# IndigoPurple/DEQSCI

Hardware: AMD Instinct MI355X
Metric: reconstructed frames/sec at 256x256x8, 180 DEQ iters (higher is better)
Workload: dtype f32 (tensors and accumulation; the 64->64 layers' products as split-fp16 MFMAs, see arithmetic)

## Files before the change

deqsci_amd/_hip.py:

```python
import ctypes
import math
import os

import torch

LAYOUT_HWB = 0
LAYOUT_BHW = 1
MAX_M = 8
PART_STRIDE = MAX_M + 1
WGRAD_CHAIN = 4096

_LIB_PATH = os.environ.get("DEQSCI_HIP_LIB") or os.path.join(os.path.dirname(os.path.abspath(__file__)), "lib", "libdeqsci_hip.so")
_lib = None

_i64, _int, _f32, _ptr = ctypes.c_int64, ctypes.c_int, ctypes.c_float, ctypes.c_void_p
_f64 = ctypes.c_double

SIGNATURES = {
    "deqsci_sci_forward_f32": [_ptr, _ptr, _ptr, _i64, _i64, _i64, _i64, _int, _int, _ptr],
    "deqsci_sci_adjoint_f32": [_ptr, _ptr, _ptr, _i64, _i64, _i64, _i64, _int, _int, _ptr],
    "deqsci_phi_sum_f32": [_ptr, _ptr, _i64, _i64, _i64, _i64, _int, _ptr],
    "deqsci_gap_update_f32": [_ptr, _ptr, _ptr, _ptr, _ptr, _i64, _i64, _i64, _i64, _int, _int, _int, _ptr],
    "deqsci_gap_update_grad_f32": [_ptr, _ptr, _ptr, _ptr, _ptr, _ptr, _ptr, _ptr, _ptr, _i64, _i64, _i64, _i64, _int, _int, _ptr],
    "deqsci_sci_mask_grad_f32": [_ptr, _ptr, _ptr, _i64, _i64, _i64, _i64, _int, _int, _ptr],
# ... 34 lines not shown
    "deqsci_conv3x3_c64_to_1_split16": [_ptr, _ptr, _ptr, _i64, _i64, _i64, _int, _ptr, _int, _ptr],
    "deqsci_conv3x3_c64_to_1_p32": [_ptr, _ptr, _ptr, _i64, _i64, _i64, _int, _ptr, _int, _ptr],
    "deqsci_conv3x3_c1_to_64_p32": [_ptr, _ptr, _ptr, _i64, _i64, _i64, _int, _ptr, _int, _ptr, _ptr],
    "deqsci_ffdnet_head_p32": [_ptr, _ptr, _ptr, _i64, _ptr, _i64, _i64, _i64, _int, _ptr, _int, _ptr, _int, _ptr],
    "deqsci_ffdnet_tail_p32": [_ptr, _ptr, _ptr, _i64, _i64, _i64, _int, _ptr, _int, _ptr],
    "deqsci_conv3x3_c1_to_64_sp16": [_ptr, _ptr, _ptr, _i64, _i64, _i64, _int, _ptr, _int, _ptr, _ptr],
    "deqsci_ssim_f32": [_ptr, _ptr, _ptr, _i64, _i64, _i64, _i64, _int, _int, _int, _int, _ptr, _ptr],
    "deqsci_sqerr_rows_f32": [_ptr, _ptr, _ptr, _i64, _i64, _i64, _int, _ptr, _ptr],
    "deqsci_gaptv_f32": [_ptr, _ptr, _ptr, _ptr, _i64, _i64, _i64, _i64, _int, _int, _f64, _f64, _f64, _int, _ptr, _ptr, _ptr],
    "deqsci_tv_chambolle_f32": [_ptr, _ptr, _i64, _i64, _i64, _f64, _f64, _int, _f64, _ptr, _ptr, _ptr],
    "deqsci_relu_mask_pack_f32": [_ptr, _ptr, _i64, _ptr],
    "deqsci_conv3x3_c64_winograd_masked_f32": [_ptr, _ptr, _ptr, _ptr, _i64, _i64, _i64, _ptr],
    "deqsci_conv3x3_c1_to_64_masked_f32": [_ptr, _ptr, _ptr, _ptr, _i64, _i64, _i64, _ptr],
    "deqsci_ffdnet_head_masked_f32": [_ptr, _ptr, _ptr, _ptr, _i64, _i64, _i64, _ptr],
    "deqsci_power_step_f32": [_ptr, _ptr, _ptr, _ptr, _i64, _i64, _ptr, _ptr],
    "deqsci_broyden_dots_f32": [_ptr, _ptr, _ptr, _ptr, _ptr, _ptr, _ptr, _i64, _i64, _int, _int, _ptr],
    "deqsci_broyden_update_f32": [_ptr, _ptr, _ptr, _ptr, _ptr, _ptr, _ptr, _ptr, _ptr, _ptr, _i64, _i64, _int, _int, _int, _ptr],
    "deqsci_epsilon2_norms_f32": [_ptr, _ptr, _ptr, _ptr, _ptr, _i64, _i64, _ptr],
    "deqsci_epsilon2_update_f32": [_ptr, _ptr, _ptr, _ptr, _ptr, _ptr, _i64, _i64, _f32, _ptr],
    "deqsci_wgrad3x3_c64_c64_f32": [_ptr, _ptr, _ptr, _i64, _i64, _i64, _ptr, _ptr],
    "deqsci_wgrad3x3_c1_c64_f32": [_ptr, _ptr, _ptr, _int, _i64, _i64, _i64, _ptr, _ptr],
    "deqsci_wgrad3x3_c64_c64_bn_f32": [_ptr, _ptr, _ptr, _ptr, _ptr, _ptr, _ptr, _i64, _i64, _i64, _ptr, _ptr],
    "deqsci_wgrad3x3_shuffle_f32": [_ptr, _ptr, _i64, _ptr, _ptr, _int, _i64, _i64, _i64, _ptr, _ptr],
    "deqsci_realsn_power_f32": [_ptr, _ptr, _ptr, _ptr, _ptr, _int, _f32, _f32, _i64, _i64, _i64, _i64, _ptr, _ptr],
    "deqsci_realsn_grad_f32": [_ptr, _ptr, _ptr, _ptr, _ptr, _ptr, _f32, _i64, _i64, _i64, _i64, _ptr, _ptr],
    "deqsci_event_create": [ctypes.POINTER(_ptr)],
    "deqsci_event_destroy": [_ptr],
    "deqsci_event_elapsed_ms": [_ptr, _ptr, ctypes.POINTER(_f32)],
}
OTHER_EXPORTS = ("deqsci_version", "deqsci_error_string", "deqsci_anderson_chunks",
                 "deqsci_partials_bytes", "deqsci_gram_bytes", "deqsci_gram_ref_bytes", "deqsci_ssim_workspace_bytes",
                 "deqsci_gaptv_workspace_bytes", "deqsci_tv_chambolle_workspace_bytes", "deqsci_sqerr_workspace_bytes", "deqsci_power_workspace_bytes",
                 "deqsci_broyden_workspace_bytes", "deqsci_broyden_chunk", "deqsci_epsilon2_workspace_bytes", "deqsci_epsilon2_chunk",
                 "deqsci_wgrad_workspace_bytes", "deqsci_wgrad_bn_workspace_bytes", "deqsci_realsn_workspace_bytes")


class DeqsciHipError(RuntimeError):
    pass


def lib_path():
    return _LIB_PATH


def load():
    global _lib
    if _lib is not None:
        return _lib
    if not os.path.exists(_LIB_PATH):
        raise DeqsciHipError(
            f"{_LIB_PATH} is missing: build it with `make` (or __graft_entry__.build()). "
            "deqsci_amd has no CPU / eager fallback for its HIP kernels.")
    lib = ctypes.CDLL(_LIB_PATH, mode=ctypes.RTLD_GLOBAL)
    for name, argtypes in SIGNATURES.items():
        fn = getattr(lib, name)
        fn.argtypes = argtypes
        fn.restype = _int
    lib.deqsci_version.restype = ctypes.c_char_p
    lib.deqsci_error_string.restype = ctypes.c_char_p
    lib.deqsci_error_string.argtypes = [_int]
    lib.deqsci_anderson_chunks.restype = _i64
    lib.deqsci_anderson_chunks.argtypes = [_i64, _i64]
    lib.deqsci_partials_bytes.restype = ctypes.c_size_t
    lib.deqsci_partials_bytes.argtypes = [_i64, _i64]
    lib.deqsci_gram_bytes.restype = ctypes.c_size_t
    lib.deqsci_gram_bytes.argtypes = [_i64]
    lib.deqsci_gram_ref_bytes.restype = ctypes.c_size_t
    lib.deqsci_gram_ref_bytes.argtypes = [_i64, _i64]
    lib.deqsci_ssim_workspace_bytes.restype = _i64
    lib.deqsci_ssim_workspace_bytes.argtypes = [_i64, _i64, _i64, _i64, _int]
    lib.deqsci_sqerr_workspace_bytes.restype = ctypes.c_size_t
    lib.deqsci_sqerr_workspace_bytes.argtypes = [_i64, _i64]
    lib.deqsci_power_workspace_bytes.restype = ctypes.c_size_t
    lib.deqsci_power_workspace_bytes.argtypes = [_i64, _i64]
    lib.deqsci_broyden_workspace_bytes.restype = ctypes.c_size_t
    lib.deqsci_broyden_workspace_bytes.argtypes = [_i64, _i64, _int]
    lib.deqsci_broyden_chunk.restype = _i64
    lib.deqsci_broyden_chunk.argtypes = []
    lib.deqsci_epsilon2_workspace_bytes.restype = ctypes.c_size_t
    lib.deqsci_epsilon2_workspace_bytes.argtypes = [_i64, _i64]
    lib.deqsci_epsilon2_chunk.restype = _i64
    lib.deqsci_epsilon2_chunk.argtypes = []
    lib.deqsci_wgrad_workspace_bytes.restype = ctypes.c_size_t
    lib.deqsci_wgrad_workspace_bytes.argtypes = [_i64, _i64, _i64]
    lib.deqsci_wgrad_bn_workspace_bytes.restype = ctypes.c_size_t
    lib.deqsci_wgrad_bn_workspace_bytes.argtypes = [_i64, _i64, _i64]
    lib.deqsci_realsn_workspace_bytes.restype = ctypes.c_size_t
    lib.deqsci_realsn_workspace_bytes.argtypes = [_i64, _i64, _i64, _i64]
    lib.deqsci_gaptv_workspace_bytes.restype = _i64
# ... 793 lines not shown

def ffdnet_head_split16(x, weights, sigma, out=None, in_rng=None, in_exp=SP16_DEFAULT_EXP, out_rng=None, out_exp=SP16_DEFAULT_EXP, track=None):
    return _ffdnet_head("ffdnet_head_split16", Sp16, x, weights, sigma, out, in_rng, in_exp, out_rng, out_exp, track)


def _ffdnet_head(what, act, x, weights, sigma, out, in_rng, in_exp, out_rng, out_exp, track=None):
    n, c, H2, W2 = x.shape
    if c != 1 or H2 % 2 or W2 % 2 or not isinstance(weights, HeadSplit16Weights):
        raise DeqsciHipError(f"{what}: (n,1,even,even) image and HeadSplit16Weights required, got {tuple(x.shape)}")
    if sigma.numel() not in (1, n) or sigma.dtype != torch.float32 or not sigma.is_cuda:
        raise DeqsciHipError(f"{what}: sigma must be a fp32 GPU tensor with 1 or n elements")
    H, W = H2 // 2, W2 // 2
    o = out if out is not None else act.empty(n, H, W, x.device)
    if not isinstance(o, act) or (o.n, o.H, o.W) != (n, H, W):
        raise DeqsciHipError(f"{what}: out must be a {act.__name__} of the output's shape")
    o.rng, o.exp = out_rng, int(out_exp)
    wp = weights.packed if weights.packed.device == x.device else weights.packed.to(x.device)
    args = (_p(x, "x"), wp.data_ptr(), sigma.data_ptr(), 0 if sigma.numel() == 1 else sigma.stride(0), o.t.data_ptr(), n, H, W, weights.sw,
            _rng(in_rng, n), int(in_exp), _rng(out_rng, n), o.exp)
    with _dev(x):
        if act is Sp16:
            _check(load().deqsci_ffdnet_head_split16(*args, _rng(track, n), _stream()), what)
        else:
            _check(load().deqsci_ffdnet_head_p32(*args, _stream()), what)
    return o


def tail_split16(h, weights, out=None):
    if not isinstance(h, Sp16):
        raise DeqsciHipError("tail_split16: an Sp16 activation and TailSplit16Weights are required")
    return _tail("tail_split16", h, weights, out)


def _tail(what, h, weights, out):
    if not isinstance(weights, TailSplit16Weights):
        raise DeqsciHipError(f"{what}: TailSplit16Weights of a (4,64,3,3) or (1,64,3,3) weight are required")
    f = 2 if weights.cout == 4 else 1
    o = out if out is not None else torch.empty((h.n, 1, f * h.H, f * h.W), device=h.t.device, dtype=torch.float32)
    wp = weights.packed if weights.packed.device == h.t.device else weights.packed.to(h.t.device)
    if isinstance(h, Sp16):
        fn = load().deqsci_ffdnet_tail_split16 if weights.cout == 4 else load().deqsci_conv3x3_c64_to_1_split16
    else:
        fn = load().deqsci_ffdnet_tail_p32 if weights.cout == 4 else load().deqsci_conv3x3_c64_to_1_p32
    with _dev(h.t):
        _check(fn(h.t.data_ptr(), wp.data_ptr(), _p(o, "out"), h.n, h.H, h.W, weights.sw, _rng(h.rng, h.n), h.exp, _stream()), what)
    return o


def conv3x3_c64_split16(x, weights, bias=None, relu=True, out=None, out_f32=False, events=None, out_rng=None, out_exp=SP16_DEFAULT_EXP,
                        track=None):
    if not isinstance(x, Sp16) or tuple(x.t.shape) != (x.n, 4, 2, 2, x.H, x.W, 8) or not x.t.is_contiguous() or x.t.dtype != torch.float16 or not x.t.is_cuda:
        raise DeqsciHipError("conv3x3_c64_split16: a contiguous Sp16 GPU activation is required")
    if not isinstance(weights, Split16Weights) or weights.packed.numel() != 4 * 9 * 2 * 2 * 64 * 8:
        raise DeqsciHipError("conv3x3_c64_split16: weights must be a Split16Weights")
    n, H, W, dev = x.n, x.H, x.W, x.t.device
    wp = weights.packed if weights.packed.device == dev else weights.packed.to(dev)
    if track is not None:
        if out_f32:
            raise DeqsciHipError("conv3x3_c64_split16: a measuring launch (track=) serves the sp16 output")
        with _dev(x.t):
            _check(load().deqsci_conv3x3_c64_split16(x.t.data_ptr(), wp.data_ptr(), _p(bias, "bias", True), None, n, H, W, 1 if relu else 0,
                                                     weights.sw, _rng(x.rng, n), x.exp, None, 0, _rng(track, n), 0, _stream(), None, None),
                   "conv3x3_c64_split16 (measuring)")
        return None
    if out_f32:
        o = out if out is not None else torch.empty((n, 64, H, W), dtype=torch.float32, device=dev, memory_format=torch.channels_last)
        ot = o
    else:
        o = out if out is not None else Sp16.empty(n, H, W, dev)
        o.rng, o.exp = out_rng, int(out_exp)
        ot = o.t
    ev = _hook_events("s16", n, H, W, events) or (None, None)
    with _dev(x.t):
        _check(load().deqsci_conv3x3_c64_split16(x.t.data_ptr(), wp.data_ptr(), _p(bias, "bias", True), ot.data_ptr(), n, H, W, 1 if relu else 0,
                                                 weights.sw, _rng(x.rng, n), x.exp, _rng(out_rng, n), int(out_exp), None, 1 if out_f32 else 0,
                                                 _stream(), ev[0], ev[1]), "conv3x3_c64_split16")
# ... 169 lines not shown
        p = torch.stack((hi, lo), 0)
        p = p.reshape(2, 3, 2, 2, 2, 32, 4, 2, 8)
        self.packed = p.permute(6, 2, 3, 1, 0, 4, 7, 5, 8).contiguous()


def _act_check(x, what):
    if (not isinstance(x, P32) or tuple(x.t.shape) != (x.n, 8, 2, x.H, -(-x.W // 64), 2, 32, 4) or x.t.dtype != torch.float32 or not x.t.is_contiguous()
            or not x.t.is_cuda):
        raise DeqsciHipError(f"{what}: a contiguous P32 GPU activation is required")


def conv3x3_c64_wino16(x, weights, bias=None, relu=True, out=None, events=None, out_rng=None, out_exp=SP16_DEFAULT_EXP):
    _act_check(x, "conv3x3_c64_wino16")
    if not isinstance(weights, Wino16Weights) or weights.packed.numel() != 4 * 2 * 2 * 3 * 2 * 2 * 64 * 8:
        raise DeqsciHipError("conv3x3_c64_wino16: weights must be a Wino16Weights")
    n, H, W, dev = x.n, x.H, x.W, x.t.device
    wp = weights.packed if weights.packed.device == dev else weights.packed.to(dev)
    o = out if out is not None else P32.empty(n, H, W, dev)
    if not isinstance(o, P32):
        raise DeqsciHipError("conv3x3_c64_wino16: out must be a P32")
    o.rng, o.exp = out_rng, int(out_exp)
    ev = _hook_events("w16", n, H, W, events) or (None, None)
    with _dev(x.t):
        _check(load().deqsci_conv3x3_c64_wino16(x.t.data_ptr(), wp.data_ptr(), _p(bias, "bias", True), o.t.data_ptr(), n, H, W, 1 if relu else 0,
                                                weights.sw, _rng(x.rng, n), x.exp, _rng(out_rng, n), int(out_exp), _stream(), ev[0], ev[1]),
               "conv3x3_c64_wino16")
    return o


def ffdnet_head_p32(x, weights, sigma, out=None, in_rng=None, in_exp=SP16_DEFAULT_EXP, out_rng=None, out_exp=SP16_DEFAULT_EXP):
    return _ffdnet_head("ffdnet_head_p32", P32, x, weights, sigma, out, in_rng, in_exp, out_rng, out_exp)


def ffdnet_tail_p32(h, weights, out=None):
    _act_check(h, "ffdnet_tail_p32")
    return _tail("ffdnet_tail_p32", h, weights, out)


def conv3x3_c64_wino16_stack(x, stack, ranges=None, events=None, per_launch=None, rng_offset=0, out_bufs=None, check=None):
    _act_check(x, "conv3x3_c64_wino16_stack")
    if not isinstance(stack, Wino16Stack):
        raise DeqsciHipError("conv3x3_c64_wino16_stack: a Wino16Stack is required")
    return _stack_launch("conv3x3_c64_wino16_stack", x, stack, ranges, events, per_launch, rng_offset, out_bufs, check)


class Wino16Stack(_Stack):
    __slots__ = ()
    ACT, WEIGHTS, TILE, HOOK, ENTRY = P32, Wino16Weights, (8, 64), "w16stack", "deqsci_conv3x3_c64_wino16_stack"
    launch = staticmethod(conv3x3_c64_wino16_stack)


class Conv64Weights:
    __slots__ = ("f22", "f44", "_w", "_s16", "_w16")

    def __init__(self, w, s16=False):
        self.f22 = pack_winograd_weights(w)
        self.f44 = pack_winograd44_weights(w)
        self._w, self._s16, self._w16 = w.detach(), None, None
        if s16:
            self._s16 = Split16Weights(self._w)
            self._w16 = Wino16Weights(self._w)

    @property
    def w16(self):
        if self._w16 is None:
            self._w16 = Wino16Weights(self._w)
        return self._w16

    @property
    def s16(self):
        if self._s16 is None:
            self._s16 = Split16Weights(self._w)
        return self._s16


def pack_conv64_weights(w, s16=False):
    return Conv64Weights(w, s16=s16)


_T_TILE_F22, _T_TILE_F44, _T_TILE_S16 = 21.5, 33.5, 29.5


# ... 370 lines not shown
```

deqsci_amd/csrc/conv_s16.hip:

```cpp
#include "common.hpp"
#include <hip/hip_ext.h>
#include <type_traits>
#pragma clang diagnostic ignored "-Winline-asm"

namespace deqsci {
namespace s16 {

typedef _Float16 h8 __attribute__((ext_vector_type(8)));
typedef _Float16 h2 __attribute__((ext_vector_type(2)));
typedef float f32x16 __attribute__((ext_vector_type(16)));
typedef float f32x4 __attribute__((ext_vector_type(4)));
typedef float f32x2 __attribute__((ext_vector_type(2)));
typedef int i32x4 __attribute__((ext_vector_type(4)));
typedef unsigned u32x4 __attribute__((ext_vector_type(4)));
typedef __attribute__((address_space(3))) char lds_char;
typedef __attribute__((address_space(3))) h8 lds_h8;

constexpr int WAVES = 8, TBW = 64 * WAVES;
constexpr int OUT_ROWS = 16, OUT_COLS = 32, RAW_ROWS = 18, RAW_COLS = 34, RAW_PIX = RAW_ROWS * RAW_COLS;
constexpr int PLANE_B = RAW_PIX * 16;
constexpr int RAW_SLOTS = 4 * RAW_PIX;
constexpr int RAW_INSTR = 5;
constexpr int RAW_BUF = WAVES * RAW_INSTR * 1024;
constexpr int W_CHUNK = 9 * 2 * 2 * 1024;
// ... 550 lines not shown
            if (colp < NCOL) {
#pragma unroll
                for (int i = 0; i < 16; ++i) P[(32 * mb + 8 * (i >> 2) + 4 * kb + (i & 3)) * PS + colp] = acc[nt][i] * oscale;
            }
        }
    }
    __syncthreads();
    const int lr = (int)threadIdx.x / TL_W, lc = (int)threadIdx.x % TL_W, r = r0 + lr, cc = c0 + lc;
    float o[COUT];
#pragma unroll
    for (int k = 0; k < COUT; ++k) o[k] = 0.0f;
#pragma unroll
    for (int tap = 0; tap < 9; ++tap) {
        const float* pp = P + ((lr + tap / 3) * TL_IW + lc + tap % 3) * PS + COUT * tap;
        if (COUT == 4) {
            const f32x4 v = *reinterpret_cast<const f32x4*>(pp);
            o[0] += v.x; o[COUT > 1 ? 1 : 0] += v.y; o[COUT > 2 ? 2 : 0] += v.z; o[COUT > 3 ? 3 : 0] += v.w;
        } else {
#pragma unroll
            for (int k = 0; k < COUT; ++k) o[k] += pp[k];
        }
    }
    if (r < H && cc < W) {
        if (COUT == 4) {
            float* op = out + (int64_t)n * 4 * H * W + (int64_t)(2 * r) * (2 * W) + 2 * cc;
            *reinterpret_cast<f32x2*>(op) = (f32x2){o[0], o[COUT > 1 ? 1 : 0]};
            *reinterpret_cast<f32x2*>(op + 2 * W) = (f32x2){o[COUT > 2 ? 2 : 0], o[COUT > 3 ? 3 : 0]};
        } else {
            out[(int64_t)n * H * W + (int64_t)r * W + cc] = o[0];
        }
    }
}


constexpr int HS_H = 8, HS_W = 32, HS_P = 2 * HS_H + 4, HS_Q = 2 * HS_W + 4, HS_QS = HS_Q + 2, HS_SW = HS_W + 2, HS_SS = HS_SW + 1;
template <int TRACK, int P32>
__global__ __launch_bounds__(256) void head_s16_kernel(const float* __restrict__ x, const char* __restrict__ Wp, const float* __restrict__ sigma,
                                                       int sigma_stride, char* __restrict__ y, int H, int W, int w_exp, const float* __restrict__ in_amax,
                                                       int in_exp, const float* __restrict__ out_amax, int out_exp, float* __restrict__ track) {
    __shared__ __attribute__((aligned(16))) unsigned patch[HS_P * HS_QS + (HS_H + 2) * HS_SS];
    __shared__ uint32_t trk_s[4];
    constexpr int SGM = HS_P * HS_QS;
    const int n = blockIdx.z, r0 = blockIdx.y * HS_H, c0 = blockIdx.x * HS_W;
    const int H2 = 2 * H, W2 = 2 * W;
    const float* xn = x + (int64_t)n * H2 * W2;
    const float sig = sigma[(int64_t)n * sigma_stride];
    const int e_in = in_amax ? sp16_act_exp(fmaxf(in_amax[n], __builtin_fabsf(sig))) : in_exp, e_out = out_amax ? sp16_act_exp(out_amax[n]) : out_exp;
    const float in_scale = sp16_pow2(e_in), oscale = sp16_pow2(e_out - e_in - w_exp);
    float tmax = 0.0f;
    auto patch_px = [&](int e) __attribute__((always_inline)) -> float {
        const int pr = e / HS_Q, pc = e - pr * HS_Q;
        const int gr = 2 * r0 - 2 + pr, gc = 2 * c0 - 2 + pc;
        return (e < HS_P * HS_Q && gr >= 0 && gr < H2 && gc >= 0 && gc < W2) ? xn[(int64_t)gr * W2 + gc] * in_scale : 0.0f;
    };
    for (int e = threadIdx.x; e < HS_P * HS_Q; e += 512) {
        const int e1 = e + 256;
        unsigned hh, ll;
        split_pair(patch_px(e), patch_px(e1), hh, ll);
        patch[(e / HS_Q) * HS_QS + e % HS_Q] = (hh & 0xffffu) | (ll << 16);
        if (e1 < HS_P * HS_Q) patch[(e1 / HS_Q) * HS_QS + e1 % HS_Q] = (hh >> 16) | (ll & 0xffff0000u);
    }
    {
        unsigned hh, ll;
        split_pair(sig * in_scale, 0.0f, hh, ll);
        const unsigned sgw = (hh & 0xffffu) | (ll << 16);
        for (int e = threadIdx.x; e < (HS_H + 2) * HS_SW; e += 256) {
// ... 204 lines not shown
extern "C" int deqsci_absmax_f32(const float* x, int64_t n, int64_t count, float* amax, deqsci_stream_t stream) {
    if (!x || !amax) return DEQSCI_ERR_NULL;
    if (count <= 0 || n <= 0) return DEQSCI_ERR_SHAPE;
    if (n > 65535) return DEQSCI_ERR_UNSUPPORTED;
    if (!aligned16(x)) return DEQSCI_ERR_ALIGN;
    int64_t blocks = ceil_div(count, 256 * 4 * 8);
    const int64_t cap = ceil_div(8 * (int64_t)num_cus(), n);
    blocks = blocks < cap ? blocks : cap;
    hipLaunchKernelGGL(s16::absmax_kernel, dim3((unsigned)(blocks < 1 ? 1 : blocks), (unsigned)n), dim3(256), 0, static_cast<hipStream_t>(stream), x, count, amax);
    return launch_status();
}

template <int COUT, int P32 = 0>
static int tail_s16_impl(const void* x_sp16, const void* w_packed, float* out, int64_t n, int64_t H, int64_t W, int w_exp, const float* in_amax,
                         int in_exp, deqsci_stream_t stream) {
    if (!x_sp16 || !w_packed || !out) return DEQSCI_ERR_NULL;
    if (n <= 0 || H <= 0 || W <= 0) return DEQSCI_ERR_SHAPE;
    if (n > 65535 || H > (1 << 20) || W > (1 << 20) || sp16_bad_exp(w_exp) || sp16_bad_exp(in_exp)) return DEQSCI_ERR_UNSUPPORTED;
    if (!aligned16(x_sp16) || !aligned16(w_packed) || !aligned16(out)) return DEQSCI_ERR_ALIGN;
    const int64_t tiles_x = ceil_div(W, s16::TL_W), tiles_y = ceil_div(H, s16::TL_H), n_tiles = n * tiles_x * tiles_y;
    if (n_tiles > (1 << 30)) return DEQSCI_ERR_UNSUPPORTED;
    const dim3 grid((unsigned)(8 * ceil_div(n_tiles, 8)));
    if (P32 && H * (64 * ceil_div(W, 64)) * 256 + 16 > (int64_t)s16::RAW_OOB) return DEQSCI_ERR_UNSUPPORTED;
    hipLaunchKernelGGL((s16::tail_s16_kernel<COUT, P32>), grid, dim3(256), 0, static_cast<hipStream_t>(stream), static_cast<const char*>(x_sp16),
                       static_cast<const char*>(w_packed), out, (int)H, (int)W, w_exp, in_amax, in_exp, (int)tiles_x, (int)tiles_y, (int)n_tiles);
    return launch_status();
}

extern "C" int deqsci_ffdnet_tail_split16(const void* x_sp16, const void* w_packed, float* out, int64_t n, int64_t H, int64_t W, int w_exp,
                                          const float* in_amax, int in_exp, deqsci_stream_t stream) {
    return tail_s16_impl<4>(x_sp16, w_packed, out, n, H, W, w_exp, in_amax, in_exp, stream);
}

extern "C" int deqsci_ffdnet_tail_p32(const void* x_p32, const void* w_packed, float* out, int64_t n, int64_t H, int64_t W, int w_exp,
                                      const float* in_amax, int in_exp, deqsci_stream_t stream) {
    return tail_s16_impl<4, 1>(x_p32, w_packed, out, n, H, W, w_exp, in_amax, in_exp, stream);
}

extern "C" int deqsci_conv3x3_c64_to_1_p32(const void* x_p32, const void* w_packed, float* out, int64_t n, int64_t H, int64_t W, int w_exp,
                                           const float* in_amax, int in_exp, deqsci_stream_t stream) {
    return tail_s16_impl<1, 1>(x_p32, w_packed, out, n, H, W, w_exp, in_amax, in_exp, stream);
}

extern "C" int deqsci_conv3x3_c64_to_1_split16(const void* x_sp16, const void* w_packed, float* out, int64_t n, int64_t H, int64_t W, int w_exp,
                                               const float* in_amax, int in_exp, deqsci_stream_t stream) {
    return tail_s16_impl<1>(x_sp16, w_packed, out, n, H, W, w_exp, in_amax, in_exp, stream);
}

template <int P32>
static int head_s16_impl(const float* x, const void* w_packed, const float* sigma, int64_t sigma_stride, void* h_out,
                         int64_t n, int64_t H, int64_t W, int w_exp, const float* in_amax, int in_exp, const float* out_amax,
                         int out_exp, float* track_amax, deqsci_stream_t stream) {
    if (!x || !w_packed || !sigma || !h_out) return DEQSCI_ERR_NULL;
    if (n <= 0 || H <= 0 || W <= 0 || sigma_stride < 0) return DEQSCI_ERR_SHAPE;
    const int64_t pitch = P32 ? 64 * ceil_div(W, 64) : W;
    if (n > 65535 || H > (1 << 20) || W > (1 << 20) || H * pitch * 256 + 16 > (int64_t)s16::RAW_OOB) return DEQSCI_ERR_UNSUPPORTED;
    if (sp16_bad_exp(w_exp) || sp16_bad_exp(in_exp) || sp16_bad_exp(out_exp)) return DEQSCI_ERR_UNSUPPORTED;
    if (!aligned16(w_packed) || !aligned16(h_out)) return DEQSCI_ERR_ALIGN;
    const dim3 grid((unsigned)ceil_div(W, s16::HS_W), (unsigned)ceil_div(H, s16::HS_H), (unsigned)n);
    if (track_amax)
        hipLaunchKernelGGL((s16::head_s16_kernel<1, P32>), grid, dim3(256), 0, static_cast<hipStream_t>(stream), x, static_cast<const char*>(w_packed), sigma,
                           (int)sigma_stride, static_cast<char*>(h_out), (int)H, (int)W, w_exp, in_amax, in_exp, out_amax, out_exp, track_amax);
    else
        hipLaunchKernelGGL((s16::head_s16_kernel<0, P32>), grid, dim3(256), 0, static_cast<hipStream_t>(stream), x, static_cast<const char*>(w_packed), sigma,
                           (int)sigma_stride, static_cast<char*>(h_out), (int)H, (int)W, w_exp, in_amax, in_exp, out_amax, out_exp, track_amax);
    return launch_status();
}

extern "C" int deqsci_ffdnet_head_split16(const float* x, const void* w_packed, const float* sigma, int64_t sigma_stride, void* h_sp16,
                                          int64_t n, int64_t H, int64_t W, int w_exp, const float* in_amax, int in_exp, const float* out_amax,
                                          int out_exp, float* track_amax, deqsci_stream_t stream) {
    return head_s16_impl<0>(x, w_packed, sigma, sigma_stride, h_sp16, n, H, W, w_exp, in_amax, in_exp, out_amax, out_exp, track_amax, stream);
}

// ... 6 lines not shown
```

deqsci_amd/csrc/conv_w16.hip:

```cpp
#include "common.hpp"
#include <hip/hip_ext.h>
#include <type_traits>
#pragma clang diagnostic ignored "-Winline-asm"

namespace deqsci {
namespace w16 {

typedef _Float16 h8 __attribute__((ext_vector_type(8)));
typedef float f32x16 __attribute__((ext_vector_type(16)));
typedef float f32x4 __attribute__((ext_vector_type(4)));
typedef float f32x2 __attribute__((ext_vector_type(2)));
typedef int i32x4 __attribute__((ext_vector_type(4)));
typedef unsigned u32x4 __attribute__((ext_vector_type(4)));
typedef __attribute__((address_space(3))) char lds_char;
typedef __attribute__((address_space(3))) u32x4 lds_u32x4;
typedef __attribute__((address_space(3))) f32x4 lds_f32x4;

constexpr int WAVES = 8, TBW = 64 * WAVES;
constexpr int OUT_ROWS = 8, OUT_COLS = 64, RAW_ROWS = 10, RAW_COLS = 66, RAW_HALF = 33, RAW_PIX = RAW_ROWS * RAW_COLS;
constexpr int PLANE_B = RAW_PIX * 16;
constexpr int RAW_SLOTS = 4 * RAW_PIX;
constexpr int RAW_TOTAL = 42;
constexpr int RAW_INSTR = 6;
constexpr int RAW_BUF = RAW_TOTAL * 1024;
// ... 466 lines not shown
static_assert(sizeof(w16::StackLayer) == 24, "the layer table of deqsci_conv3x3_c64_wino16_stack is three 8-byte words per layer");

extern "C" int deqsci_conv3x3_c64_wino16(const void* x_p32, const void* u_packed, const float* bias, void* y_p32, int64_t n, int64_t H, int64_t W,
                                         int relu, int w_exp, const float* in_amax, int in_exp, const float* out_amax, int out_exp,
                                         deqsci_stream_t stream, void* start_event, void* stop_event) {
    if (!x_p32 || !u_packed || !y_p32) return DEQSCI_ERR_NULL;
    if ((start_event == nullptr) != (stop_event == nullptr)) return DEQSCI_ERR_NULL;
    if (n <= 0 || H <= 0 || W <= 0) return DEQSCI_ERR_SHAPE;
    if (x_p32 == y_p32 || sp16_bad_exp(w_exp) || sp16_bad_exp(in_exp) || sp16_bad_exp(out_exp)) return DEQSCI_ERR_UNSUPPORTED;
    if (!aligned16(x_p32) || !aligned16(u_packed) || !aligned16(y_p32)) return DEQSCI_ERR_ALIGN;
    const int64_t tiles_x = ceil_div(W, w16::OUT_COLS), tiles_y = ceil_div(H, w16::OUT_ROWS);
    const int64_t n_tiles = n * tiles_x * tiles_y;
    if (n_tiles > (int64_t)INT32_MAX / 16 || H * tiles_x * w16::OUT_COLS * 256 + 16 > (int64_t)w16::RAW_OOB) return DEQSCI_ERR_UNSUPPORTED;
    hipStream_t st = static_cast<hipStream_t>(stream);
    const int64_t resident = (int64_t)num_cus();
    const dim3 grid((unsigned)(n_tiles < resident ? n_tiles : resident));
    uint32_t mg_img, sh_img, mg_tx, sh_tx;
    mdiv_magic((uint32_t)(tiles_x * tiles_y), &mg_img, &sh_img);
    mdiv_magic((uint32_t)tiles_x, &mg_tx, &sh_tx);
    hipEvent_t ev0 = static_cast<hipEvent_t>(start_event), ev1 = static_cast<hipEvent_t>(stop_event);
    hipExtLaunchKernelGGL((w16::conv_w16_kernel<0>), grid, dim3(w16::TBW), 0, st, ev0, ev1, 0, static_cast<const char*>(x_p32), static_cast<const char*>(u_packed),
                          bias, static_cast<char*>(y_p32), (int)H, (int)W, relu, w_exp, in_amax, in_exp, out_amax, out_exp, (int)tiles_x,
                          (int)tiles_y, (int)n_tiles, mg_img, sh_img, mg_tx, sh_tx, static_cast<char*>(nullptr),
                          static_cast<const w16::StackLayer*>(nullptr), 1, static_cast<unsigned*>(nullptr), 0);
    return launch_status();
}

extern "C" int deqsci_conv3x3_c64_wino16_stack(const void* x_p32, void* y_even, void* y_odd, const void* layers, int n_layers,
                                               int64_t n, int64_t H, int64_t W, const float* ranges, int64_t range_stride, int in_exp, int out_exp,
                                               void* flags, deqsci_stream_t stream, void* start_event, void* stop_event) {
    if (!x_p32 || !y_even || !layers || !flags || (n_layers > 1 && !y_odd)) return DEQSCI_ERR_NULL;
    if ((start_event == nullptr) != (stop_event == nullptr)) return DEQSCI_ERR_NULL;
    if (n <= 0 || H <= 0 || W <= 0 || n_layers <= 0 || (ranges && (range_stride < n || range_stride > INT32_MAX))) return DEQSCI_ERR_SHAPE;
    if (x_p32 == y_even || x_p32 == y_odd || y_even == y_odd || n_layers > 64 || sp16_bad_exp(in_exp) || sp16_bad_exp(out_exp)) return DEQSCI_ERR_UNSUPPORTED;
    if (!aligned16(x_p32) || !aligned16(y_even) || !aligned16(y_odd) || (reinterpret_cast<uintptr_t>(layers) & 7u) || (reinterpret_cast<uintptr_t>(flags) & 3u))
        return DEQSCI_ERR_ALIGN;
    const int64_t tiles_x = ceil_div(W, w16::OUT_COLS), tiles_y = ceil_div(H, w16::OUT_ROWS);
    const int64_t n_tiles = n * tiles_x * tiles_y;
    if (H * tiles_x * w16::OUT_COLS * 256 + 16 > (int64_t)w16::RAW_OOB) return DEQSCI_ERR_UNSUPPORTED;
    if (n_tiles > (int64_t)INT32_MAX / (16 * 32)) return DEQSCI_ERR_UNSUPPORTED;
    static int occ_cache[64] = {0};
    const int64_t fit = resident_workgroups(w16::conv_w16_kernel<1>, w16::TBW, occ_cache);
    if (fit <= 0) return DEQSCI_ERR_UNSUPPORTED;
    const int64_t resident = fit < (int64_t)num_cus() ? fit : (int64_t)num_cus();
    hipStream_t st = static_cast<hipStream_t>(stream);
    uint32_t mg_img, sh_img, mg_tx, sh_tx;
    mdiv_magic((uint32_t)(tiles_x * tiles_y), &mg_img, &sh_img);
    mdiv_magic((uint32_t)tiles_x, &mg_tx, &sh_tx);
    hipEvent_t ev0 = static_cast<hipEvent_t>(start_event), ev1 = static_cast<hipEvent_t>(stop_event);
    hipExtLaunchKernelGGL((w16::conv_w16_kernel<1>), dim3((unsigned)(n_tiles < resident ? n_tiles : resident)), dim3(w16::TBW), 0, st, ev0, ev1, 0,
                          static_cast<const char*>(x_p32), static_cast<const char*>(nullptr), static_cast<const float*>(nullptr), static_cast<char*>(y_even),
                          (int)H, (int)W, 0, 0, ranges, in_exp, static_cast<const float*>(nullptr), out_exp, (int)tiles_x, (int)tiles_y, (int)n_tiles,
                          mg_img, sh_img, mg_tx, sh_tx, static_cast<char*>(y_odd), static_cast<const w16::StackLayer*>(layers), n_layers,
                          static_cast<unsigned*>(flags), (int)range_stride);
    return launch_status();
}
```

deqsci_amd/engine.py:

```python
import math
import numpy as np

import torch
import torch.nn.functional as F

from . import _hip
from ._hip import LAYOUT_BHW, LAYOUT_HWB
from .layers import _fold_bn, conv_stack

SIGMA0 = 60 / 255
SIGMA_DECAY = 0.971


def sigma_schedule(n):
    out = np.empty(n, dtype=np.float32)
    s = np.float32(SIGMA0)
    d = np.float32(SIGMA_DECAY)
    for i in range(n):
        out[i] = s
        s = np.float32(s * d)
    return out


def _exhaust(gen):
# ... 16 lines not shown
        out.append(int(k))
    if not out:
        return None
    lo = 3 if iterator == "anderson" else 1
    for a, b in zip(out, out[1:]):
        if b <= a:
            raise ValueError(f"snapshots={tuple(out)}: must be strictly increasing")
    if out[0] < lo:
        raise ValueError(f"snapshots={tuple(out)}: the smallest horizon of the {iterator} iteration is {lo}")
    if out[-1] >= max_iter:
        raise ValueError(f"snapshots={tuple(out)}: every horizon must be smaller than max_iter={max_iter} (the run's own result is the last one)")
    return tuple(out)


class _Edges:
    __slots__ = ("div", "ffdnet", "relu", "head_w", "tail_w", "head_w16", "tail_w16")

    def __init__(self, div=1, relu=True):
        self.div, self.ffdnet, self.relu = div, div == 2, relu
        self.head_w = self.tail_w = self.head_w16 = self.tail_w16 = None

    def head(self, x, sigma, act=None, out=None, in_rng=None, out_rng=None, out_exp=_hip.SP16_DEFAULT_EXP, track=None):
        if not self.ffdnet:
            return _hip.conv3x3_c1_to_64(x, self.head_w, relu=self.relu, out=out, sp16=act is _hip.Sp16, p32=act is _hip.P32,
                                         out_rng=out_rng, out_exp=out_exp, track=track)
        if act is None:
            return _hip.ffdnet_head(x, self.head_w, sigma)
        if act is _hip.P32:
            return _hip.ffdnet_head_p32(x, self.head_w16, sigma, out, in_rng, out_rng=out_rng, out_exp=out_exp)
        return _hip.ffdnet_head_split16(x, self.head_w16, sigma, out, in_rng, out_rng=out_rng, out_exp=out_exp, track=track)

    def tail(self, h, out=None, in_bias=None):
        if isinstance(h, _hip.P32):
            return _hip.ffdnet_tail_p32(h, self.tail_w16, out)
        if isinstance(h, _hip.Sp16):
            return _hip.tail_split16(h, self.tail_w16, out)
        return (_hip.ffdnet_tail if self.ffdnet else _hip.conv3x3_c64_to_1)(h.contiguous(memory_format=torch.channels_last), self.tail_w, out, in_bias)


class _Denoiser:

    def __init__(self, net, fold_bn=True, channels_last=None, fused_epilogue=True, fused_edges=True, winograd=True, conv64="fast",
                 act_range="data", blk32=True, stack=True, stack_kernel="w16"):
        from .networks import FFDNet
        self.net = net
        if stack_kernel not in ("w16", "s16"):
            raise ValueError(f"stack_kernel={stack_kernel!r}: expected 'w16' or 's16'")
        self.stack_kernel = stack_kernel
        self.gate = None
        self.per_layer_w16 = False
        self.last_path = None
        self._wstacks = {}
        self.stack = bool(stack)
        self.stack_per_launch = None
        self.slice_edges = True
        self._stacks = {}
        self.stack_launches = 0
        self.fused_edges = fused_edges
        self.winograd = winograd
        self.conv64 = conv64
        self.f22_calls = None
        self._policy = conv64
        self.blk32 = bool(blk32)
        if act_range not in ("data", "fixed"):
            raise ValueError(f"act_range={act_range!r}: expected 'data' or 'fixed'")
        self.act_range = act_range
        self.ranges = None
# ... 802 lines not shown
```

include/deqsci_hip.h:

```cpp
#ifndef DEQSCI_HIP_H
#define DEQSCI_HIP_H

#include <stddef.h>
#include <stdint.h>

#ifdef __cplusplus
extern "C" {
#endif

#define DEQSCI_LAYOUT_HWB 0
#define DEQSCI_LAYOUT_BHW 1

#define DEQSCI_MAX_M 8
#define DEQSCI_PART_STRIDE (DEQSCI_MAX_M + 1)

#define DEQSCI_ERR_NULL        (-1)
#define DEQSCI_ERR_SHAPE       (-2)
#define DEQSCI_ERR_ALIGN       (-3)
#define DEQSCI_ERR_UNSUPPORTED (-4)

typedef void* deqsci_stream_t;

const char* deqsci_version(void);
const char* deqsci_error_string(int code);
// ... 113 lines not shown
                               deqsci_stream_t stream, void* start_event, void* stop_event);
int deqsci_conv3x3_c64_split16_stack(const void* x_sp16, void* y_even, void* y_odd, const void* layers, int n_layers,
                                     int64_t n, int64_t H, int64_t W, const float* ranges, int64_t range_stride, int in_exp, int out_exp,
                                     void* flags, deqsci_stream_t stream, void* start_event, void* stop_event);
int deqsci_conv3x3_c64_wino16(const void* x_p32, const void* u_packed, const float* bias, void* y_p32,
                              int64_t n, int64_t H, int64_t W, int relu, int w_exp, const float* in_amax, int in_exp,
                              const float* out_amax, int out_exp,
                              deqsci_stream_t stream, void* start_event, void* stop_event);
int deqsci_conv3x3_c64_wino16_stack(const void* x_p32, void* y_even, void* y_odd, const void* layers, int n_layers,
                                    int64_t n, int64_t H, int64_t W, const float* ranges, int64_t range_stride, int in_exp, int out_exp,
                                    void* flags, deqsci_stream_t stream, void* start_event, void* stop_event);
int deqsci_f32_to_split16(const float* x_nhwc, void* y_sp16, int64_t n, int64_t H, int64_t W, const float* amax, int exp,
                          deqsci_stream_t stream);
int deqsci_absmax_f32(const float* x, int64_t n, int64_t count, float* amax, deqsci_stream_t stream);
int deqsci_conv3x3_c1_to_64_sp16(const float* x, const float* w_packed, void* h_sp16, int64_t n, int64_t H, int64_t W, int relu,
                                 const float* out_amax, int out_exp, float* track_amax, deqsci_stream_t stream);
int deqsci_conv3x3_c1_to_64_p32(const float* x, const float* w_packed, void* h_p32, int64_t n, int64_t H, int64_t W, int relu,
                                const float* out_amax, int out_exp, float* track_amax, deqsci_stream_t stream);
int deqsci_conv3x3_c64_to_1_p32(const void* x_p32, const void* w_packed, float* out, int64_t n, int64_t H, int64_t W,
                                int w_exp, const float* in_amax, int in_exp, deqsci_stream_t stream);
int deqsci_ffdnet_tail_split16(const void* x_sp16, const void* w_packed, float* out, int64_t n, int64_t H, int64_t W,
                               int w_exp, const float* in_amax, int in_exp, deqsci_stream_t stream);
int deqsci_conv3x3_c64_to_1_split16(const void* x_sp16, const void* w_packed, float* out, int64_t n, int64_t H, int64_t W,
                                    int w_exp, const float* in_amax, int in_exp, deqsci_stream_t stream);
int deqsci_ffdnet_head_split16(const float* x, const void* w_packed, const float* sigma, int64_t sigma_stride, void* h_sp16,
                               int64_t n, int64_t H, int64_t W, int w_exp, const float* in_amax, int in_exp,
                               const float* out_amax, int out_exp, float* track_amax, deqsci_stream_t stream);

int deqsci_ffdnet_head_p32(const float* x, const void* w_packed, const float* sigma, int64_t sigma_stride, void* h_p32,
                           int64_t n, int64_t H, int64_t W, int w_exp, const float* in_amax, int in_exp,
                           const float* out_amax, int out_exp, deqsci_stream_t stream);
int deqsci_ffdnet_tail_p32(const void* x_p32, const void* w_packed, float* out, int64_t n, int64_t H, int64_t W,
                           int w_exp, const float* in_amax, int in_exp, deqsci_stream_t stream);

int64_t deqsci_ssim_workspace_bytes(int64_t M, int64_t H, int64_t W, int64_t B, int layout);
int deqsci_ssim_f32(const float* x, const float* y, double* out, int64_t M, int64_t H, int64_t W, int64_t B,
                    int layout, int window, int valid, int clamp_x, void* workspace, deqsci_stream_t stream);

size_t deqsci_sqerr_workspace_bytes(int64_t bsz, int64_t N);
int deqsci_sqerr_rows_f32(const float* x, const float* gt, double* out, int64_t bsz, int64_t N, int64_t x_stride, int clamp_x,
                          void* workspace, deqsci_stream_t stream);

int64_t deqsci_gaptv_workspace_bytes(int64_t bsz, int64_t H, int64_t W, int64_t B);
int deqsci_gaptv_f32(const float* y, const float* phi, const float* phi_sum, float* out, int64_t bsz, int64_t H, int64_t W,
                     int64_t B, int phi_shared, int maxiter, double step, double weight, double eps, int n_iter_max, int* stop,
                     void* workspace, deqsci_stream_t stream);
int64_t deqsci_tv_chambolle_workspace_bytes(int64_t n, int64_t H, int64_t W);
int deqsci_tv_chambolle_f32(const float* image, float* out, int64_t n, int64_t H, int64_t W, double weight, double eps,
                            int n_iter_max, double tau, int* stop, void* workspace, deqsci_stream_t stream);

int deqsci_relu_mask_pack_f32(const float* a, uint64_t* mask, int64_t n_pixels, deqsci_stream_t stream);
int deqsci_conv3x3_c64_winograd_masked_f32(const float* x, const float* u_packed, const uint64_t* mask, float* y,
                                           int64_t n, int64_t H, int64_t W, deqsci_stream_t stream);
int deqsci_conv3x3_c1_to_64_masked_f32(const float* x, const float* w_packed, const uint64_t* mask, float* h,
                                       int64_t n, int64_t H, int64_t W, deqsci_stream_t stream);

int deqsci_ffdnet_head_masked_f32(const float* x, const float* w_packed, const uint64_t* mask, float* h,
                                  int64_t n, int64_t H, int64_t W, deqsci_stream_t stream);
size_t deqsci_power_workspace_bytes(int64_t bsz, int64_t N);
int deqsci_power_step_f32(const float* w, const float* v_prev, float* v_out, double* table_row, int64_t bsz, int64_t N,
                          void* workspace, deqsci_stream_t stream);

#define DEQSCI_BROYDEN_MAX_L 27
#define DEQSCI_BROYDEN_TABLE_STRIDE 84
int64_t deqsci_broyden_chunk(void);
size_t deqsci_broyden_workspace_bytes(int64_t bsz, int64_t N, int L);
// ... 55 lines not shown
```

Measured before the change: 151.5.

## Add row-streaming persistent tail kernel for P32 FFDNet tail with ring buffer

Adds a persistent, XCD-aware tail kernel for the P32 path. Each workgroup walks 16-row by 128-column bands and keeps the MFMA-produced per-tap partial products in a six-row shared-memory ring, so the 3x3 output reduction reuses rows across steps instead of recomputing tile halos. A heuristic picks between this rows form and the existing tiles kernel based on how well the band count fills the CUs, and explicit _rows/_tiles entry points are exposed. Separately, the Wino16 stack's head buffer now aliases the stack's odd output buffer to save a separate allocation, with the C check relaxed to allow this.

```diff
diff --git a/deqsci_amd/_hip.py b/deqsci_amd/_hip.py
--- a/deqsci_amd/_hip.py
+++ b/deqsci_amd/_hip.py
@@ -90,7 +90,8 @@
                  "deqsci_partials_bytes", "deqsci_gram_bytes", "deqsci_gram_ref_bytes", "deqsci_ssim_workspace_bytes",
                  "deqsci_gaptv_workspace_bytes", "deqsci_tv_chambolle_workspace_bytes", "deqsci_sqerr_workspace_bytes", "deqsci_power_workspace_bytes",
                  "deqsci_broyden_workspace_bytes", "deqsci_broyden_chunk", "deqsci_epsilon2_workspace_bytes", "deqsci_epsilon2_chunk",
-                 "deqsci_wgrad_workspace_bytes", "deqsci_wgrad_bn_workspace_bytes", "deqsci_realsn_workspace_bytes")
+                 "deqsci_wgrad_workspace_bytes", "deqsci_wgrad_bn_workspace_bytes", "deqsci_realsn_workspace_bytes") + tuple(
+                     base + form for base in ("deqsci_ffdnet_tail_p32", "deqsci_conv3x3_c64_to_1_p32") for form in ("_rows", "_tiles"))
 
 
 class DeqsciHipError(RuntimeError):
@@ -113,6 +114,10 @@
     for name, argtypes in SIGNATURES.items():
         fn = getattr(lib, name)
         fn.argtypes = argtypes
+        fn.restype = _int
+    for name in OTHER_EXPORTS[-4:]:
+        fn = getattr(lib, name)
+        fn.argtypes = SIGNATURES[name.rsplit("_", 1)[0]]
         fn.restype = _int
     lib.deqsci_version.restype = ctypes.c_char_p
     lib.deqsci_error_string.restype = ctypes.c_char_p
@@ -972,7 +977,12 @@
     return _tail("tail_split16", h, weights, out)
 
 
-def _tail(what, h, weights, out):
+TAIL_P32_FORM = None
+
+
+def _tail(what, h, weights, out, form=None):
+    if form not in (None, "rows", "tiles") or (form is not None and isinstance(h, Sp16)):
+        raise DeqsciHipError(f"{what}: form must be None, 'rows' or 'tiles', and only a P32 input has forms")
     if not isinstance(weights, TailSplit16Weights):
         raise DeqsciHipError(f"{what}: TailSplit16Weights of a (4,64,3,3) or (1,64,3,3) weight are required")
     f = 2 if weights.cout == 4 else 1
@@ -981,7 +991,7 @@
     if isinstance(h, Sp16):
         fn = load().deqsci_ffdnet_tail_split16 if weights.cout == 4 else load().deqsci_conv3x3_c64_to_1_split16
     else:
-        fn = load().deqsci_ffdnet_tail_p32 if weights.cout == 4 else load().deqsci_conv3x3_c64_to_1_p32
+        fn = getattr(load(), ("deqsci_ffdnet_tail_p32" if weights.cout == 4 else "deqsci_conv3x3_c64_to_1_p32") + ("" if form is None else "_" + form))
     with _dev(h.t):
         _check(fn(h.t.data_ptr(), wp.data_ptr(), _p(o, "out"), h.n, h.H, h.W, weights.sw, _rng(h.rng, h.n), h.exp, _stream()), what)
     return o
@@ -1217,9 +1227,9 @@
     return _ffdnet_head("ffdnet_head_p32", P32, x, weights, sigma, out, in_rng, in_exp, out_rng, out_exp)
 
 
-def ffdnet_tail_p32(h, weights, out=None):
+def ffdnet_tail_p32(h, weights, out=None, form=None):
     _act_check(h, "ffdnet_tail_p32")
-    return _tail("ffdnet_tail_p32", h, weights, out)
+    return _tail("ffdnet_tail_p32", h, weights, out, form)
 
 
 def conv3x3_c64_wino16_stack(x, stack, ranges=None, events=None, per_launch=None, rng_offset=0, out_bufs=None, check=None):
@@ -1229,10 +1239,18 @@
     return _stack_launch("conv3x3_c64_wino16_stack", x, stack, ranges, events, per_launch, rng_offset, out_bufs, check)
 
 
+STACK_HEAD_ALIAS = True
+
+
 class Wino16Stack(_Stack):
     __slots__ = ()
     ACT, WEIGHTS, TILE, HOOK, ENTRY = P32, Wino16Weights, (8, 64), "w16stack", "deqsci_conv3x3_c64_wino16_stack"
     launch = staticmethod(conv3x3_c64_wino16_stack)
+
+    def head_buffer(self, n, H, W):
+        if STACK_HEAD_ALIAS and self.n_layers >= 2:
+            return self.state(n, H, W)[1]
+        return super().head_buffer(n, H, W)
 
 
 class Conv64Weights:
diff --git a/deqsci_amd/csrc/conv_s16.hip b/deqsci_amd/csrc/conv_s16.hip
--- a/deqsci_amd/csrc/conv_s16.hip
+++ b/deqsci_amd/csrc/conv_s16.hip
@@ -606,6 +606,177 @@
     }
 }
 
+constexpr int TR_R = 16, TR_SW = 128, TR_RING = 6, TR_STEPS = TR_R / 2 + 1, TR_D = 2, TR_TB = 512;
+static_assert(TR_RING == 6 && TR_R % 2 == 0, "a step reads four ring rows while the next one writes the other two");
+template <int COUT>
+__global__ __launch_bounds__(TR_TB) void tail_rows_kernel(const char* __restrict__ x, const char* __restrict__ Wp, float* __restrict__ out, int H, int W,
+                                                          int w_exp, const float* __restrict__ in_amax, int in_exp, int strips, int bands_y, int n_bands) {
+    constexpr int NCOL = 9 * COUT, NT = (NCOL + 31) / 32, PS = NCOL, ROWF = (TR_SW + 2) * PS;
+    __shared__ __attribute__((aligned(16))) float P[TR_RING * ROWF];
+    const int tid = (int)threadIdx.x, lane = tid & 63, wave = __builtin_amdgcn_readfirstlane(tid >> 6), pl = lane & 31, kb = lane >> 5;
+    const int half = wave >> 2, b64 = (wave & 3) >> 1, par = wave & 1;
+    const int lcol = 64 * b64 + 2 * pl + par;
+    const int Wq = 64 * ((W + 63) / 64);
+    const int64_t HW = (int64_t)H * Wq;
+    const uint32_t lane_off = (uint32_t)(((int64_t)(2 * kb) * HW + pl) * 16);
+    const int ring_col = (64 * b64 + 2 * (4 * kb) + par + 1) * PS;
+    h8 Bw[4][2][NT];
+#pragma unroll
+    for (int c = 0; c < 4; ++c)
+#pragma unroll
+        for (int hl = 0; hl < 2; ++hl)
+#pragma unroll
+            for (int nt = 0; nt < NT; ++nt) Bw[c][hl][nt] = *reinterpret_cast<const h8*>(Wp + ((((c * 2 + hl) * NT + nt) * 64 + lane) * 16));
+
+    auto split = [&](const f32x4 (&raw)[8], h8 (&A)[4][2]) __attribute__((always_inline)) {
+#pragma unroll
+        for (int c = 0; c < 4; ++c) {
+            const float v[8] = {raw[2 * c].x, raw[2 * c].y, raw[2 * c].z, raw[2 * c].w, raw[2 * c + 1].x, raw[2 * c + 1].y, raw[2 * c + 1].z, raw[2 * c + 1].w};
+#pragma unroll
+            for (int k = 0; k < 8; ++k) {
+                const _Float16 hh = (_Float16)v[k];
+                A[c][0][k] = hh;
+                A[c][1][k] = (_Float16)(v[k] - (float)hh);
+            }
+        }
+    };
+    auto mma = [&](const h8 (&A)[4][2], f32x16 (&acc)[NT]) __attribute__((always_inline)) {
+#pragma unroll
+        for (int nt = 0; nt < NT; ++nt)
+#pragma unroll
+            for (int i = 0; i < 16; ++i) acc[nt][i] = 0.0f;
+#pragma unroll
+        for (int c = 0; c < 4; ++c)
+#pragma unroll
+            for (int nt = 0; nt < NT; ++nt) {
+                acc[nt] = __builtin_amdgcn_mfma_f32_32x32x16_f16(A[c][1], Bw[c][0][nt], acc[nt], 0, 0, 0);
+                acc[nt] = __builtin_amdgcn_mfma_f32_32x32x16_f16(A[c][0], Bw[c][1][nt], acc[nt], 0, 0, 0);
+            }
+#pragma unroll
+        for (int c = 0; c < 4; ++c)
+#pragma unroll
+            for (int nt = 0; nt < NT; ++nt) acc[nt] = __builtin_amdgcn_mfma_f32_32x32x16_f16(A[c][0], Bw[c][0][nt], acc[nt], 0, 0, 0);
+    };
+
+    if (strips == 1 && wave == 0) {
+        h8 A[4][2];
+#pragma unroll
+        for (int c = 0; c < 4; ++c) A[c][0] = A[c][1] = (h8){0, 0, 0, 0, 0, 0, 0, 0};
+        f32x16 acc[NT];
+        mma(A, acc);
+#pragma unroll
+        for (int nt = 0; nt < NT; ++nt) {
+            const int colp = 32 * nt + pl;
+            if (colp < NCOL)
+                for (int sl = 0; sl < TR_RING; ++sl) P[sl * ROWF + (kb ? (Wq + 1) * PS : 0) + colp] = acc[nt][0];
+        }
+    }
+
+    const int per_xcd = (n_bands + 7) >> 3, wg_xcd = (int)gridDim.x >> 3;
+    const int t_first = ((int)blockIdx.x & 7) * per_xcd, t_end = t_first + per_xcd < n_bands ? t_first + per_xcd : n_bands;
+    for (int t = t_first + ((int)blockIdx.x >> 3); t < t_end; t += wg_xcd) {
+        const int n = t / (strips * bands_y), rt = t - n * (strips * bands_y), sx = rt / bands_y, by = rt - sx * bands_y;
+        const int r0 = by * TR_R, c0 = sx * TR_SW, hb = H - r0 < TR_R ? H - r0 : TR_R;
+        const int nb = (Wq - c0) >> 6 < 2 ? (Wq - c0) >> 6 : 2;
+        const bool active = b64 < nb;
+        const float oscale = sp16_pow2(-(in_amax ? sp16_act_exp(in_amax[n]) : in_exp) - w_exp);
+        const char* xn = x + (int64_t)n * HW * 256;
+        const uint32_t col_off = (uint32_t)(c0 + (active ? 64 * b64 : 0) + 32 * par) * 16u + lane_off, plane_b = (uint32_t)HW * 16u;
+        const bool col_ok = active && c0 + lcol < W;
+        auto fetch = [&](int s, f32x4 (&raw)[8]) __attribute__((always_inline)) {
+            const int gr = r0 - 1 + 2 * s + half, grc = gr < 0 ? 0 : gr >= H ? H - 1 : gr;
+            const uint32_t row_off = (uint32_t)(grc * Wq) * 16u + col_off;
+#pragma unroll
+            for (int k = 0; k < 8; ++k)
+                raw[k] = *reinterpret_cast<const f32x4*>(xn + (row_off + (uint32_t)(4 * (k >> 1) + (k & 1)) * plane_b));
+        };
+        auto zero = [&](int s, f32x4 (&raw)[8]) __attribute__((always_inline)) {
+            const int gr = r0 - 1 + 2 * s + half;
+            const bool ok = col_ok && gr >= 0 && gr < H;
+#pragma unroll
+            for (int k = 0; k < 8; ++k) raw[k] = ok ? raw[k] : (f32x4){0, 0, 0, 0};
+        };
+        f32x4 raw[TR_D][8];
+#pragma unroll
+        for (int d = 0; d < TR_D; ++d) fetch(d, raw[d]);
+#pragma unroll
+        for (int s = 0; s < TR_STEPS; ++s) {
+            if (2 * s >= hb + 2) break;
+            float* Prow = P + ((2 * s) % TR_RING + half) * ROWF;
+            {
+                h8 A[4][2];
+                zero(s, raw[s % TR_D]);
+                split(raw[s % TR_D], A);
+                if (s + TR_D < TR_STEPS) fetch(s + TR_D, raw[s % TR_D]);
+                f32x16 acc[NT];
+                mma(A, acc);
+#pragma unroll
+                for (int nt = 0; nt < NT; ++nt) {
+                    const int colp = 32 * nt + pl;
+                    if (colp < (active ? NCOL : 0)) {
+#pragma unroll
+                        for (int i = 0; i < 16; ++i) Prow[ring_col + 2 * (8 * (i >> 2) + (i & 3)) * PS + colp] = acc[nt][i] * oscale;
+                    }
+                }
+            }
+            if (strips > 1 && (wave & 3) == 0) {
+                const int gr = r0 - 1 + 2 * s + half, gc = pl == 0 ? c0 - 1 : c0 + 64 * nb;
+                const bool ok = pl < 2 && gr >= 0 && gr < H && gc >= 0 && gc < W;
+                const int grc = gr < 0 ? 0 : gr >= H ? H - 1 : gr, gcc = ok ? gc : 0;
+                const uint32_t off = lane_off - (uint32_t)pl * 16u + (uint32_t)(grc * Wq + (gcc & ~63) + ((gcc & 1) << 5) + ((gcc & 63) >> 1)) * 16u;
+                const uint32_t keep = ok ? ~0u : 0u;
+                f32x4 rh[8];
+#pragma unroll
+                for (int k = 0; k < 8; ++k) {
+                    const u32x4 v = *reinterpret_cast<const u32x4*>(xn + (off + (uint32_t)(4 * (k >> 1) + (k & 1)) * plane_b));
+                    rh[k] = __builtin_bit_cast(f32x4, v & keep);
+                }
+                h8 A[4][2];
+                split(rh, A);
+                f32x16 acc[NT];
+                mma(A, acc);
+#pragma unroll
+                for (int nt = 0; nt < NT; ++nt) {
+                    const int colp = 32 * nt + pl;
+                    if (colp < NCOL && kb == 0) {
+                        Prow[colp] = acc[nt][0] * oscale;
+                        Prow[(64 * nb + 1) * PS + colp] = acc[nt][1] * oscale;
+                    }
+                }
+            }
+            __syncthreads();
+            if (s >= 1) {
+                constexpr int SPLIT = COUT == 4 ? 2 : 1, OC = COUT / SPLIT;
+                const int i2 = tid % SPLIT, col = (tid / SPLIT) & (TR_SW - 1), jr = tid / (SPLIT * TR_SW), j = 2 * s - 2 + jr;
+                const int r = r0 + j, cc = c0 + col;
+                if (jr < 2 && j < hb && cc < W) {
+                    float o[OC];
+#pragma unroll
+                    for (int k = 0; k < OC; ++k) o[k] = 0.0f;
+#pragma unroll
+                    for (int tap = 0; tap < 9; ++tap) {
+                        int sl = (2 * s - 2) % TR_RING + jr + tap / 3;
+                        sl = sl >= TR_RING ? sl - TR_RING : sl;
+                        const float* pp = P + sl * ROWF + (col + tap % 3) * PS + COUT * tap + OC * i2;
+                        if (COUT == 4) {
+                            const f32x2 v = *reinterpret_cast<const f32x2*>(pp);
+                            o[0] += v.x; o[OC > 1 ? 1 : 0] += v.y;
+                        } else {
+#pragma unroll
+                            for (int k = 0; k < OC; ++k) o[k] += pp[k];
+                        }
+                    }
+                    if (COUT == 4)
+                        *reinterpret_cast<f32x2*>(out + (int64_t)n * 4 * H * W + (int64_t)(2 * r + i2) * (2 * W) + 2 * cc) = (f32x2){o[0], o[OC > 1 ? 1 : 0]};
+                    else
+                        out[(int64_t)n * H * W + (int64_t)r * W + cc] = o[0];
+                }
+            }
+        }
+        __syncthreads();
+    }
+}
+
 
 constexpr int HS_H = 8, HS_W = 32, HS_P = 2 * HS_H + 4, HS_Q = 2 * HS_W + 4, HS_QS = HS_Q + 2, HS_SW = HS_W + 2, HS_SS = HS_SW + 1;
 template <int TRACK, int P32>
@@ -876,14 +1047,49 @@
     return tail_s16_impl<4>(x_sp16, w_packed, out, n, H, W, w_exp, in_amax, in_exp, stream);
 }
 
+template <int COUT>
+static int tail_p32_impl(const void* x_p32, const void* w_packed, float* out, int64_t n, int64_t H, int64_t W, int w_exp, const float* in_amax,
+                         int in_exp, deqsci_stream_t stream, int form) {
+    if (!x_p32 || !w_packed || !out) return DEQSCI_ERR_NULL;
+    if (n <= 0 || H <= 0 || W <= 0) return DEQSCI_ERR_SHAPE;
+    if (n > 65535 || H > (1 << 20) || W > (1 << 20) || sp16_bad_exp(w_exp) || sp16_bad_exp(in_exp)) return DEQSCI_ERR_UNSUPPORTED;
+    const int64_t strips = ceil_div(W, s16::TR_SW), bands_y = ceil_div(H, s16::TR_R), n_bands = n * strips * bands_y;
+    const int64_t cus = num_cus() >= 8 ? num_cus() / 8 * 8 : 8;
+    if (form == 0) form = (n_bands <= (1 << 30) && 4 * n_bands >= 3 * ceil_div(n_bands, cus) * cus) ? 1 : 2;
+    if (form == 2) return tail_s16_impl<COUT, 1>(x_p32, w_packed, out, n, H, W, w_exp, in_amax, in_exp, stream);
+    if (!aligned16(x_p32) || !aligned16(w_packed) || !aligned16(out)) return DEQSCI_ERR_ALIGN;
+    if (n_bands > (1 << 30) || H * (64 * ceil_div(W, 64)) * 256 + 16 > (int64_t)s16::RAW_OOB) return DEQSCI_ERR_UNSUPPORTED;
+    const int64_t want = 8 * ceil_div(n_bands, 8);
+    hipLaunchKernelGGL((s16::tail_rows_kernel<COUT>), dim3((unsigned)(want < cus ? want : cus)), dim3(s16::TR_TB), 0, static_cast<hipStream_t>(stream),
+                       static_cast<const char*>(x_p32), static_cast<const char*>(w_packed), out, (int)H, (int)W, w_exp, in_amax, in_exp, (int)strips,
+                       (int)bands_y, (int)n_bands);
+    return launch_status();
+}
+
 extern "C" int deqsci_ffdnet_tail_p32(const void* x_p32, const void* w_packed, float* out, int64_t n, int64_t H, int64_t W, int w_exp,
                                       const float* in_amax, int in_exp, deqsci_stream_t stream) {
-    return tail_s16_impl<4, 1>(x_p32, w_packed, out, n, H, W, w_exp, in_amax, in_exp, stream);
+    return tail_p32_impl<4>(x_p32, w_packed, out, n, H, W, w_exp, in_amax, in_exp, stream, 0);
+}
+extern "C" int deqsci_ffdnet_tail_p32_rows(const void* x_p32, const void* w_packed, float* out, int64_t n, int64_t H, int64_t W, int w_exp,
+                                           const float* in_amax, int in_exp, deqsci_stream_t stream) {
+    return tail_p32_impl<4>(x_p32, w_packed, out, n, H, W, w_exp, in_amax, in_exp, stream, 1);
+}
+extern "C" int deqsci_ffdnet_tail_p32_tiles(const void* x_p32, const void* w_packed, float* out, int64_t n, int64_t H, int64_t W, int w_exp,
+                                            const float* in_amax, int in_exp, deqsci_stream_t stream) {
+    return tail_p32_impl<4>(x_p32, w_packed, out, n, H, W, w_exp, in_amax, in_exp, stream, 2);
 }
 
 extern "C" int deqsci_conv3x3_c64_to_1_p32(const void* x_p32, const void* w_packed, float* out, int64_t n, int64_t H, int64_t W, int w_exp,
                                            const float* in_amax, int in_exp, deqsci_stream_t stream) {
-    return tail_s16_impl<1, 1>(x_p32, w_packed, out, n, H, W, w_exp, in_amax, in_exp, stream);
+    return tail_p32_impl<1>(x_p32, w_packed, out, n, H, W, w_exp, in_amax, in_exp, stream, 0);
+}
+extern "C" int deqsci_conv3x3_c64_to_1_p32_rows(const void* x_p32, const void* w_packed, float* out, int64_t n, int64_t H, int64_t W, int w_exp,
+                                                const float* in_amax, int in_exp, deqsci_stream_t stream) {
+    return tail_p32_impl<1>(x_p32, w_packed, out, n, H, W, w_exp, in_amax, in_exp, stream, 1);
+}
+extern "C" int deqsci_conv3x3_c64_to_1_p32_tiles(const void* x_p32, const void* w_packed, float* out, int64_t n, int64_t H, int64_t W, int w_exp,
+                                                 const float* in_amax, int in_exp, deqsci_stream_t stream) {
+    return tail_p32_impl<1>(x_p32, w_packed, out, n, H, W, w_exp, in_amax, in_exp, stream, 2);
 }
 
 extern "C" int deqsci_conv3x3_c64_to_1_split16(const void* x_sp16, const void* w_packed, float* out, int64_t n, int64_t H, int64_t W, int w_exp,
diff --git a/deqsci_amd/csrc/conv_w16.hip b/deqsci_amd/csrc/conv_w16.hip
--- a/deqsci_amd/csrc/conv_w16.hip
+++ b/deqsci_amd/csrc/conv_w16.hip
@@ -522,7 +522,8 @@
     if (!x_p32 || !y_even || !layers || !flags || (n_layers > 1 && !y_odd)) return DEQSCI_ERR_NULL;
     if ((start_event == nullptr) != (stop_event == nullptr)) return DEQSCI_ERR_NULL;
     if (n <= 0 || H <= 0 || W <= 0 || n_layers <= 0 || (ranges && (range_stride < n || range_stride > INT32_MAX))) return DEQSCI_ERR_SHAPE;
-    if (x_p32 == y_even || x_p32 == y_odd || y_even == y_odd || n_layers > 64 || sp16_bad_exp(in_exp) || sp16_bad_exp(out_exp)) return DEQSCI_ERR_UNSUPPORTED;
+    if (x_p32 == y_even || (x_p32 == y_odd && n_layers < 2) || y_even == y_odd || n_layers > 64 || sp16_bad_exp(in_exp) || sp16_bad_exp(out_exp))
+        return DEQSCI_ERR_UNSUPPORTED;
     if (!aligned16(x_p32) || !aligned16(y_even) || !aligned16(y_odd) || (reinterpret_cast<uintptr_t>(layers) & 7u) || (reinterpret_cast<uintptr_t>(flags) & 3u))
         return DEQSCI_ERR_ALIGN;
     const int64_t tiles_x = ceil_div(W, w16::OUT_COLS), tiles_y = ceil_div(H, w16::OUT_ROWS);
diff --git a/deqsci_amd/engine.py b/deqsci_amd/engine.py
--- a/deqsci_amd/engine.py
+++ b/deqsci_amd/engine.py
@@ -72,7 +72,7 @@
 
     def tail(self, h, out=None, in_bias=None):
         if isinstance(h, _hip.P32):
-            return _hip.ffdnet_tail_p32(h, self.tail_w16, out)
+            return _hip.ffdnet_tail_p32(h, self.tail_w16, out, form=_hip.TAIL_P32_FORM)
         if isinstance(h, _hip.Sp16):
             return _hip.tail_split16(h, self.tail_w16, out)
         return (_hip.ffdnet_tail if self.ffdnet else _hip.conv3x3_c64_to_1)(h.contiguous(memory_format=torch.channels_last), self.tail_w, out, in_bias)
diff --git a/include/deqsci_hip.h b/include/deqsci_hip.h
--- a/include/deqsci_hip.h
+++ b/include/deqsci_hip.h
@@ -169,6 +169,14 @@
                            const float* out_amax, int out_exp, deqsci_stream_t stream);
 int deqsci_ffdnet_tail_p32(const void* x_p32, const void* w_packed, float* out, int64_t n, int64_t H, int64_t W,
                            int w_exp, const float* in_amax, int in_exp, deqsci_stream_t stream);
+int deqsci_ffdnet_tail_p32_rows(const void* x_p32, const void* w_packed, float* out, int64_t n, int64_t H, int64_t W,
+                                int w_exp, const float* in_amax, int in_exp, deqsci_stream_t stream);
+int deqsci_ffdnet_tail_p32_tiles(const void* x_p32, const void* w_packed, float* out, int64_t n, int64_t H, int64_t W,
+                                 int w_exp, const float* in_amax, int in_exp, deqsci_stream_t stream);
+int deqsci_conv3x3_c64_to_1_p32_rows(const void* x_p32, const void* w_packed, float* out, int64_t n, int64_t H, int64_t W,
+                                     int w_exp, const float* in_amax, int in_exp, deqsci_stream_t stream);
+int deqsci_conv3x3_c64_to_1_p32_tiles(const void* x_p32, const void* w_packed, float* out, int64_t n, int64_t H, int64_t W,
+                                      int w_exp, const float* in_amax, int in_exp, deqsci_stream_t stream);
 
 int64_t deqsci_ssim_workspace_bytes(int64_t M, int64_t H, int64_t W, int64_t B, int layout);
 int deqsci_ssim_f32(const float* x, const float* y, double* out, int64_t M, int64_t H, int64_t W, int64_t B,
```

Result: no change. 151.8, median of 6 (+0.3%).
